# toverainc/willow-inference-server

Measured on NVIDIA H100. Metric: Whisper large-v2 realtime multiple (audio s / s), beam 5, 3.84 s utterance, higher is better.
Workload: dtype f16

## Files before the change

willow_inference_server_b200/csrc/decoder.cuh:

```cuda
#pragma once
#include "common.cuh"
#include "kernels.h"

namespace wisb {

constexpr int DEC_MAX_ROWS = 8;
constexpr int MAX_BEAM = 8;
constexpr int MAX_CAND = 2 * MAX_BEAM;
constexpr int TOPK_CHUNKS = 32;

struct DecState {
  int pos;
  int gen_step;
  int n_done;
  int all_done;
  int ticket;
};

enum GemvEpi : int {
  GV_STORE = 0,
  GV_RESID = 1,
  GV_GELU = 2,
  GV_QKV = 3,
};
// ... 114 lines not shown
  const float* next_g = nullptr;
};
struct MegaLayer {
  MegaGemv qkv, o, cq, co, fc1, fc2;
  const __half* ck = nullptr;
  const __half* cv = nullptr;
  __half* kcache = nullptr;
  __half* vcache = nullptr;
};
struct MegaArgs {
  const MegaLayer* layers = nullptr;
  int n_layers = 0;
  MegaGemv vocab;
  int with_logits = 0;
  int R = 0, d = 0, H = 0, n_utt = 0, beam = 0, t_max = 0;
  int pf_len = 0, pf_tok_stride = 0, pf_slot_stride = 0;
  const int* tokens = nullptr;
  const __half* tok_emb = nullptr;
  const float* pos_emb = nullptr;
  float* x = nullptr;
  float* q = nullptr;
  float* ctx = nullptr;
  __half* ctx16 = nullptr;
  __half* q16 = nullptr;
  __half* xn16 = nullptr;
  float* xstat = nullptr;
  const int* indir0 = nullptr;
  const int* indir1 = nullptr;
  const int* flip = nullptr;
  const DecState* st = nullptr;
  float* cross_part = nullptr;
  unsigned* cross_flags = nullptr;
  unsigned* flags = nullptr;
  unsigned* epoch_base = nullptr;
  int barrier_mode = 0;
  int tc = 0;
  int dbg = 0;
  int trace_cta = 0, trace_layer = 0, trace_cap = 0;
  unsigned long long* trace = nullptr;
};
size_t mega_flags_words();
int mega_k_chunks(int K);
void mega_chunk_major(const __half* src, __half* dst, int N, int K, cudaStream_t stream);
void mega_mma_image(const __half* src, __half* dst, int N, int K, int grid, cudaStream_t stream);
void mega_ln_fold(const __half* w, const float* g, const float* b, const float* bias, float* s2, float* biasf, int N, int K,
                  cudaStream_t stream);
void dec_pass_run(const MegaArgs& a, int num_sms, cudaStream_t stream);

void lang_probs_run(const float* logits, long long ldl, const int* lang_ids, int n_lang, int n_utt, int row_stride,
                    float* probs , cudaStream_t stream);

}
```

willow_inference_server_b200/csrc/decoder_mega.cu:

```cuda
#include <cooperative_groups.h>

#include "decoder.cuh"
#include "ptx.cuh"

namespace wisb {

namespace {

constexpr int MG_CONS_WARPS = 7;
constexpr int MG_CONS = MG_CONS_WARPS * 32;
constexpr int MG_THREADS = MG_CONS + 32;
constexpr int MG_KC_MAX = 1536;
constexpr int MG_STAGE_BYTES = 12 * MG_KC_MAX * 2;
constexpr int MG_NSTAGE = 2;
constexpr int MG_CA_KEYS_MAX = MG_STAGE_BYTES / 128;
constexpr int MG_SCRATCH = 29696;
constexpr int MG_SLOT_BYTES = MG_CONS_WARPS * 448 * 2;
constexpr int MG_LY_STRIDE = 704;
constexpr int MG_LY_BYTES = 2 * MG_LY_STRIDE;
constexpr int MG_RED_FLOATS = (2 * 2 + 1) * MG_CONS_WARPS * 32;
constexpr int MG_SMEM = MG_NSTAGE * MG_STAGE_BYTES + 1024 + MG_RED_FLOATS * 4 + 4224 + MG_SCRATCH + MG_SLOT_BYTES + MG_LY_BYTES;
static_assert(MG_SMEM <= 232448, "decoder pass: shared memory");
static_assert(sizeof(MegaLayer) % 16 == 0 && sizeof(MegaLayer) <= MG_LY_STRIDE, "layer descriptor is copied with 16-byte cp.async");
__host__ __device__ constexpr int mg_gp(int nr) { return 32 / nr < 6 ? 32 / nr : 6; }
// ... 831 lines not shown
  if (blockIdx.x == 0 && ctid == 0) {
    *A.epoch_base = epoch;
    A.epoch_base[8] = epoch * gridDim.x;
  }
}


constexpr int FUSED_B_OFF = 36864;
template <int NR>
struct MmaSmem {
  static constexpr int NS = NR <= 5 ? 4 : 3;
  static constexpr int B_BYTES = (5120 / 64) * NR * 128;
  static constexpr int B_MIN = FUSED_B_OFF + 20 * NR * 128;
  static constexpr int B_ALLOC = B_BYTES > B_MIN ? (B_BYTES > MG_SCRATCH ? B_BYTES : MG_SCRATCH) : (B_MIN > MG_SCRATCH ? B_MIN : MG_SCRATCH);
  static constexpr int OFF_B = NS * MG_STAGE_BYTES;
  static constexpr int OFF_PART = OFF_B + B_ALLOC;
  static constexpr int PART_BYTES = MG_CONS_WARPS * 8 * 68 * 4;
  static constexpr int OFF_BARS = OFF_PART + PART_BYTES;
  static constexpr int OFF_STAT = OFF_BARS + 256;
  static constexpr int OFF_SLOT = OFF_STAT + 4224;
  static constexpr int OFF_LY = OFF_SLOT + MG_SLOT_BYTES;
  static constexpr int OFF_GEOM = OFF_LY + MG_LY_BYTES;
  static constexpr int TOTAL = OFF_GEOM + 5 * 64;
  static constexpr int STAT_OFF = 24576;
  static_assert(TOTAL <= 232448, "warp-MMA decoder pass: shared memory");
  static_assert(20 * NR * 128 <= STAT_OFF && STAT_OFF + 160 * NR * 8 <= FUSED_B_OFF && FUSED_B_OFF + 20 * NR * 128 <= B_ALLOC,
                "statistics landing zone / fused-phase B operand");
};
constexpr int MM_GROUP_ROWS = 64;
constexpr int MM_PART_LD = 68;

struct MmaGeom {
  int lo, hi, rows_pad, n_full, tail;
  int units_full, kbu_full, units_tail, kbu_tail, pad[7];
};
static_assert(sizeof(MmaGeom) == 64, "geometry table stride");
__device__ __forceinline__ void mma_units(int rows, int kblocks, int& units, int& kbu) {
  const int max_kbu = MG_STAGE_BYTES / (rows * 128);
  units = (kblocks + max_kbu - 1) / max_kbu;
  kbu = (kblocks + units - 1) / units;
}
__device__ __forceinline__ MmaGeom mma_geom(int N, int K) {
  MmaGeom m;
  const int G = static_cast<int>(gridDim.x), b = static_cast<int>(blockIdx.x);
  const int base = N / G, rem = N - base * G;
  m.lo = b * base + min(b, rem);
  m.rows_pad = base + (b < rem ? 1 : 0);
  m.hi = m.lo + m.rows_pad;
  m.n_full = m.rows_pad / MM_GROUP_ROWS;
  m.tail = m.rows_pad - m.n_full * MM_GROUP_ROWS;
  m.units_full = m.kbu_full = m.units_tail = m.kbu_tail = 0;
  if (m.n_full > 0) mma_units(MM_GROUP_ROWS, K / 64, m.units_full, m.kbu_full);
  if (m.tail > 0) mma_units(m.tail, K / 64, m.units_tail, m.kbu_tail);
  return m;
}

template <int NS>
__device__ __forceinline__ void produce_gemv_mma(Ring& rg, const MegaGemv& g, const MmaGeom* s_geom, int dbg) {
  const MmaGeom mg = s_geom[g.shape];
  const int n_groups = mg.n_full + (mg.tail ? 1 : 0);
  const int kblocks = g.K / 64;
  const uint64_t pol = l2_policy_evict_first();
  for (int gi = 0; gi < n_groups; ++gi) {
    const bool full = gi < mg.n_full;
    const int rows = full ? MM_GROUP_ROWS : mg.tail;
    const int units = full ? mg.units_full : mg.units_tail, kbu = full ? mg.kbu_full : mg.kbu_tail;
    const __half* base = g.w + static_cast<long long>(mg.lo + gi * MM_GROUP_ROWS) * g.K;
    for (int u = 0; u < units; ++u) {
      const int kb0 = u * kbu, nkb = min(kbu, kblocks - kb0);
      const int st = rg.unit % NS;
      mbar_wait(rg.empty(st), ((rg.unit / NS) & 1u) ^ 1u);
      uint32_t bytes = static_cast<uint32_t>(nkb * rows * 128);
      if (dbg & 2) bytes = (bytes >> 2) & ~15u;
      mbar_arrive_expect_tx(rg.full(st), bytes);
      bulk_load_1d_hint(rg.data0 + st * MG_STAGE_BYTES, base + static_cast<long long>(kb0) * rows * 64, bytes, rg.full(st), pol);
      ++rg.unit;
    }
  }
}

// ... 29 lines not shown
#pragma unroll
    for (int ks = 0; ks < 4; ++ks) {
      uint32_t af[NMT][4], ag[NMT][4];
#pragma unroll
      for (int m = 0; m < NMT; ++m) {
        ldmatrix_x4(a_kb + sw[ks] + m * 2048, af[m]);
        ldmatrix_x4(a_kb + a_step + sw[ks] + m * 2048, ag[m]);
      }
#pragma unroll
      for (int m = 0; m < NMT; ++m) {
        mma_m16n8k16(acc[m], af[m], bf[2 * ks], bf[2 * ks + 1]);
        mma_m16n8k16(acc2[m], ag[m], bg[2 * ks], bg[2 * ks + 1]);
      }
    }
  }
  if (it < n_it) {
    const uint4 b01 = lds128(b_kb), b23 = lds128(b_kb + b_plane);
    const uint32_t bf[8] = {b01.x, b01.y, b01.z, b01.w, b23.x, b23.y, b23.z, b23.w};
#pragma unroll
    for (int ks = 0; ks < 4; ++ks) {
      uint32_t af[NMT][4];
#pragma unroll
      for (int m = 0; m < NMT; ++m) ldmatrix_x4(a_kb + sw[ks] + m * 2048, af[m]);
#pragma unroll
      for (int m = 0; m < NMT; ++m) mma_m16n8k16(acc[m], af[m], bf[2 * ks], bf[2 * ks + 1]);
    }
  }
#pragma unroll
  for (int m = 0; m < NMT; ++m)
#pragma unroll
    for (int i = 0; i < 4; ++i) acc[m][i] += acc2[m][i];
}

constexpr int SA_WARPS = 2;
__device__ __forceinline__ void consume_self_attn_mma(const MegaArgs& A, const MegaLayer& ly, int ctid, uint8_t* s_scr,
                                                   const unsigned short* s_slot_tab, int pos_dec, int flipv, int* s_tr) {
  const int lane = ctid & 31, warp = ctid >> 5;
  const int d = A.d, H = A.H, G = static_cast<int>(gridDim.x);
  const int n_tasks = A.R * H;
  const bool pf = A.pf_len > 0;
  trace_ev(A, ctid, s_tr, 20);
  if (warp >= SA_WARPS) return;
  const uint32_t sK = smem_u32(s_scr) + warp * 8192, sV = sK + 4096;
  const unsigned short* my_slots = s_slot_tab + warp * 448;
  const __half* kcache = ly.kcache;
  const __half* vcache = ly.vcache;
  const int gq = lane >> 2, tq = lane & 3;
  const int ld_key = lane >> 3, ld_c = lane & 7;
  const uint32_t lm_off = static_cast<uint32_t>(((lane & 7) + ((lane >> 3) & 1) * 8) * 128);
  const int lm_c = lane >> 4;
  for (int i = warp; i * G + static_cast<int>(blockIdx.x) < n_tasks; i += SA_WARPS) {
    const int task = i * G + static_cast<int>(blockIdx.x);
    const bool tab = i == warp;
    const int r = task / H, h = task - r * H;
    const int pos = pf ? r % A.pf_len : pos_dec;
    const int own = row_slot(A, r);
    const int* indir = (flipv ? A.indir1 : A.indir0) + static_cast<long long>(r) * A.t_max;
    uint32_t aq[4][2];
    {
      const __half* qr = A.q16 + (static_cast<long long>(h) * A.R + r) * HEAD_DIM + 2 * tq;
#pragma unroll
      for (int ks = 0; ks < 4; ++ks) {
        aq[ks][0] = gq == 0 ? __ldcg(reinterpret_cast<const unsigned*>(qr + 16 * ks)) : 0u;
        aq[ks][1] = gq == 0 ? __ldcg(reinterpret_cast<const unsigned*>(qr + 16 * ks + 8)) : 0u;
      }
    }
    float m_run = -INFINITY, l_run = 0.f;
    float o[8][4];
#pragma unroll
    for (int j = 0; j < 8; ++j)
#pragma unroll
      for (int q = 0; q < 4; ++q) o[j][q] = 0.f;
    for (int t0 = 0; t0 <= pos; t0 += 32) {
#pragma unroll
      for (int it = 0; it < 8; ++it) {
        const int key = it * 4 + ld_key;
        const int t = min(t0 + key, pos);
        int slot = own;
        if (!pf && t != pos) slot = tab ? static_cast<int>(my_slots[t]) : __ldcg(indir + t);
        const long long off = (static_cast<long long>(slot) * A.t_max + t) * d + h * HEAD_DIM + ld_c * 8;
        const uint32_t dst = key * 128 + ((ld_c ^ (key & 7)) << 4);
        cp_async16(sK + dst, kcache + off);
        cp_async16(sV + dst, vcache + off);
      }
      cp_async_wait_all();
      __syncwarp();
      trace_ev(A, ctid, s_tr, 21);
// ... 98 lines not shown
      if (rl.bytes2 != 0) bulk_load_1d(s_b_addr + stat_off, rl.src2, rl.bytes2, xbar);
    }
  }
  cons_sync();
  if (A.trace != nullptr && blockIdx.x == 0 && ctid == 0) A.trace[2 * (epoch - epoch0)] = globaltimer_ns();
}
__device__ __forceinline__ Reload gemv_reload(const MegaArgs& A, const MegaGemv& g, const MmaGeom* s_geom) {
  Reload rl;
  if (s_geom[g.shape].rows_pad != 0) {
    rl.src = g.x16;
    rl.bytes = static_cast<uint32_t>((g.K / 64) * A.R * 128);
    if (g.ln_s2 != nullptr) {
      rl.src2 = A.xstat;
      rl.bytes2 = static_cast<uint32_t>(gridDim.x * A.R * 8);
    }
  }
  return rl;
}


template <int NR>
__device__ __forceinline__ void consume_gemv_mma(Ring& rg, const MegaArgs& A, const MegaGemv& g_mem, const MegaLayer* ly, int ctid,
                                             uint8_t* s_b, float* s_lnstat, float* s_mpart, float* s_xown, int* s_tr,
                                             const MmaGeom* s_geom, uint32_t xbar, unsigned& x_count) {
  using SM = MmaSmem<NR>;
  constexpr int NS = SM::NS;
  const MegaGemv g = g_mem;
  const MmaGeom mg = s_geom[g.shape];
  if (mg.rows_pad == 0) return;
  const int lane = ctid & 31, warp = ctid >> 5;
  const int R = A.R;
  const int kblocks = g.K / 64;
  const bool ln = g.ln_s2 != nullptr;
  const int G = static_cast<int>(gridDim.x);
  trace_ev(A, ctid, s_tr, 1);
  constexpr int NSLOT = (NR * MM_GROUP_ROWS + MG_CONS - 1) / MG_CONS;
  const int n_groups = mg.n_full + (mg.tail ? 1 : 0);
  const int first_rows = mg.n_full > 0 ? MM_GROUP_ROWS : mg.tail;
  const int wsh = (n_groups == 1 && first_rows <= 16) ? 4 : 6;
  float e_bias[NSLOT], e_s2[NSLOT], e_gain[NSLOT];
  auto prefetch_epi = [&](int gi, int rows) {
#pragma unroll
    for (int j = 0; j < NSLOT; ++j) {
      const int idx = ctid + j * MG_CONS;
      const int m = idx & ((1 << wsh) - 1), n = mg.lo + gi * MM_GROUP_ROWS + m;
      const bool ok = (idx >> wsh) < R && m < rows && n < mg.hi;
      e_bias[j] = (ok && g.bias != nullptr) ? __ldg(g.bias + n) : 0.f;
      e_s2[j] = (ok && ln) ? __ldg(g.ln_s2 + n) : 0.f;
      e_gain[j] = (ok && g.next_g != nullptr) ? __ldg(g.next_g + n) : 0.f;
    }
  };
  prefetch_epi(0, first_rows);
  const int gq = lane >> 2, tq = lane & 3;
  const int brow = gq < R ? gq : R - 1;
  const uint32_t b_lane = smem_u32(s_b) + (brow * 4 + tq) * 16, b_plane = static_cast<uint32_t>(R * 64);
  const int a_row = (lane & 7) + ((lane >> 3) & 1) * 8;
  uint32_t sw[4];
#pragma unroll
  for (int ks = 0; ks < 4; ++ks) sw[ks] = ((2 * ks + (lane >> 4)) ^ (a_row & 7)) << 4;
  const uint32_t a_lane = rg.data0 + a_row * 128;
  unsigned unit = rg.unit;
  unsigned st = unit % NS, par = (unit / NS) & 1u;
  mbar_wait(xbar, x_count & 1u);
  ++x_count;
  trace_ev(A, ctid, s_tr, 2);
  for (int gi = 0; gi < n_groups; ++gi) {
    const bool full = gi < mg.n_full;
    const int rows = full ? MM_GROUP_ROWS : mg.tail;
    const int n_mt = (rows + 15) >> 4;
    const int units = full ? mg.units_full : mg.units_tail, kbu = full ? mg.kbu_full : mg.kbu_tail;
    if (gi > 0) prefetch_epi(gi, rows);
    float acc[4][4];
#pragma unroll
    for (int m = 0; m < 4; ++m)
#pragma unroll
      for (int i = 0; i < 4; ++i) acc[m][i] = 0.f;
    int kb_next = warp;
    for (int u = 0, kb0 = 0; u < units; ++u, kb0 += kbu) {
      const int nkb = min(kbu, kblocks - kb0);
      mbar_wait(rg.full(st), par);
      if (u == 0 && gi == 0) trace_ev(A, ctid, s_tr, 3);
// ... 45 lines not shown
    for (int j = 0; j < NSLOT; ++j) {
      const int idx = ctid + j * MG_CONS;
      const int r = idx >> wsh, m = idx & ((1 << wsh) - 1);
      const int n = mg.lo + gi * MM_GROUP_ROWS + m;
      const bool valid = r < R && m < rows && n < mg.hi;
      float v = 0.f;
      if (valid) {
#pragma unroll
        for (int w = 0; w < MG_CONS_WARPS; ++w) v += s_mpart[(w * 8 + r) * MM_PART_LD + m];
        if (ln) {
          const float mean = s_lnstat[2 * r] / g.K;
          const float rstd = rsqrtf(fmaxf(s_lnstat[2 * r + 1] / g.K - mean * mean, 0.f) + 1e-5f);
          v = rstd * (v - mean * e_s2[j]);
        }
        v += e_bias[j];
      }
      if (g.epi == GV_RESID) {
        float nv = 0.f;
        if (valid) {
          nv = s_xown[r * 16 + (n - mg.lo)] + v;
          s_xown[r * 16 + (n - mg.lo)] = nv;
        }
        if (j == 0 || (idx >> 5) * 32 < R * 16) publish_resid(A, r, n, valid, nv, e_gain[j], lane);
      } else if (valid) {
        switch (g.epi) {
          case GV_STORE:
            if (g.out16 != nullptr) g.out16[(static_cast<long long>(n >> 6) * R + r) * HEAD_DIM + (n & 63)] = __float2half_rn(v * 0.125f);
            else g.out[static_cast<long long>(r) * g.ldo + n] = v;
            break;
          case GV_GELU:
            g.out16[act16_off(R, r, n)] = __float2half_rn(gelu_erf(v));
            break;
          case GV_QKV: {
            const int d = A.d;
            if (n < d) {
              A.q16[(static_cast<long long>(n >> 6) * R + r) * HEAD_DIM + (n & 63)] = __float2half_rn(v * 0.125f);
            } else {
              const int pos = row_pos(A, r);
              __half* cache = (n < 2 * d) ? ly->kcache : ly->vcache;
              const int e = (n < 2 * d) ? n - d : n - 2 * d;
              cache[(static_cast<long long>(row_slot(A, r)) * A.t_max + pos) * d + e] = __float2half_rn(v);
            }
            break;
          }
          default:
            break;
        }
      }
    }
    if (gi + 1 < n_groups) cons_sync();
  }
  trace_ev(A, ctid, s_tr, 6);
  rg.unit = unit;
}

template <int NS>
__device__ __forceinline__ void produce_cross_fused(Ring& rg, const MegaArgs& A, const MegaLayer& ly, const MmaGeom* s_geom) {
  const CrossGeom cg = cross_geom(A.n_utt, A.H);
  const uint64_t pol = l2_policy_evict_first();
  const int kblocks = A.d / 64, units = s_geom[4].units_full, kbu = s_geom[4].kbu_full;
  for (int task = blockIdx.x; task < cg.n_tasks; task += gridDim.x) {
    const int split = task % cg.S, uh = task / cg.S;
    const int h = uh % A.H;
    const __half* wq = ly.cq.w + static_cast<long long>(h) * 64 * A.d;
    for (int u = 0; u < units; ++u) {
      const int kb0 = u * kbu, nkb = min(kbu, kblocks - kb0);
      const int st = rg.unit % NS;
      mbar_wait(rg.empty(st), ((rg.unit / NS) & 1u) ^ 1u);
      mbar_arrive_expect_tx(rg.full(st), static_cast<uint32_t>(nkb * 64 * 128));
      bulk_load_1d_hint(rg.data0 + st * MG_STAGE_BYTES, wq + static_cast<long long>(kb0) * 64 * 64, static_cast<uint32_t>(nkb * 64 * 128),
                        rg.full(st), pol);
      ++rg.unit;
    }
// ... 217 lines not shown
  extern __shared__ __align__(1024) uint8_t mg_smem[];
  uint8_t* s_b = mg_smem + SM::OFF_B;
  float* s_part = reinterpret_cast<float*>(s_b);
  float* s_mpart = reinterpret_cast<float*>(mg_smem + SM::OFF_PART);
  uint64_t* bars = reinterpret_cast<uint64_t*>(mg_smem + SM::OFF_BARS);
  float* s_stat = reinterpret_cast<float*>(mg_smem + SM::OFF_STAT);
  float* s_lnstat = s_stat;
  unsigned short* s_slot_tab = reinterpret_cast<unsigned short*>(mg_smem + SM::OFF_SLOT);
  MegaLayer* s_ly = reinterpret_cast<MegaLayer*>(mg_smem + SM::OFF_LY);
  MmaGeom* s_geom = reinterpret_cast<MmaGeom*>(mg_smem + SM::OFF_GEOM);
  float* s_xown = s_stat + 784;
  int* s_tr = reinterpret_cast<int*>(s_stat + 16);
  Ring rg;
  rg.data = mg_smem;
  rg.data0 = smem_u32(mg_smem);
  rg.full0 = smem_u32(bars);
  rg.empty0 = rg.full0 + 8 * NS;
  rg.unit = 0;
  const uint32_t xbar = rg.full0 + 8 * (2 * NS);
  unsigned x_count = 0;
  const int tid = threadIdx.x;
  if ((smem_u32(mg_smem) & 1023u) != 0) __trap();
  if (tid == 0) {
    for (int s = 0; s < NS; ++s) {
      mbar_init(rg.full(s), 1);
      mbar_init(rg.empty(s), MG_CONS_WARPS);
    }
    mbar_init(xbar, 1);
    fence_mbar_init();
  }
  if (tid < 5) {
    const int d = A.d;
    const int Ns[5] = {3 * d, d, 4 * d, d, A.vocab.N}, Ks[5] = {d, d, d, 4 * d, d};
    s_geom[tid] = mma_geom(Ns[tid], Ks[tid]);
  }
  __syncthreads();
  const int L = A.n_layers;

  if (tid >= MG_CONS) {
    if (tid == MG_CONS) {
      for (int l = 0; l <= L; ++l) {
        if (l == L) {
          if (A.with_logits) produce_gemv_mma<NS>(rg, A.vocab, s_geom, A.dbg);
          break;
        }
        const MegaLayer& ly = A.layers[l];
        for (int j = 0; j < 6; ++j) {
          if (j == 2) produce_cross_fused<NS>(rg, A, ly, s_geom);
          else produce_gemv_mma<NS>(rg, (&ly.qkv)[j], s_geom, A.dbg);
        }
      }
    }
    return;
  }
  const int ctid = tid;
  unsigned epoch = *A.epoch_base;
  const unsigned epoch0 = epoch;
  if (ctid == 0) s_tr[0] = -1;
  if (A.trace != nullptr && blockIdx.x == 0 && ctid == 0) A.trace[0] = globaltimer_ns();
  auto prefetch_layer = [&](int l) {
    if (ctid < static_cast<int>(sizeof(MegaLayer) / 16))
      cp_async16(smem_u32(reinterpret_cast<uint8_t*>(s_ly) + (l & 1) * MG_LY_STRIDE) + ctid * 16,
                 reinterpret_cast<const uint8_t*>(A.layers + l) + ctid * 16);
  };
  if (L > 0) prefetch_layer(0);
  const int pos_dec = A.pf_len > 0 ? 0 : A.st->pos;
  const int flipv = *A.flip;
  if (A.pf_len == 0 && (ctid >> 5) < SA_WARPS) {
    const int task = (ctid >> 5) * static_cast<int>(gridDim.x) + static_cast<int>(blockIdx.x);
    if (task < A.R * A.H) {
      const int* indir = (flipv ? A.indir1 : A.indir0) + static_cast<long long>(task / A.H) * A.t_max;
      for (int t = ctid & 31; t < pos_dec; t += 32) s_slot_tab[(ctid >> 5) * 448 + t] = static_cast<unsigned short>(indir[t]);
    }
  }
  cp_async_wait_all();
  {
    const MmaGeom mg = s_geom[1];
    const float* gain0 = L > 0 ? A.layers[0].qkv.ln_g : A.vocab.ln_g;
    for (int base = 0; base < A.R * 16; base += MG_CONS) {
      const int idx = base + ctid;
      const int r = idx >> 4, c = idx & 15, n = mg.lo + c;
      const bool valid = r < A.R && n < mg.hi;
      float v = 0.f, gain = 0.f;
      if (valid) {
        v = __half2float(A.tok_emb[static_cast<long long>(row_token(A, r)) * A.d + n]) + A.pos_emb[static_cast<long long>(row_pos(A, r)) * A.d + n];
        gain = __ldg(gain0 + n);
        s_xown[r * 16 + c] = v;
      }
      if ((idx >> 5) * 32 < A.R * 16) publish_resid(A, r, n, valid, v, gain, ctid & 31);
    }
  }
  const uint32_t sba = smem_u32(s_b);
  Reload rl_next = L > 0 ? gemv_reload(A, A.layers[0].qkv, s_geom) : (A.with_logits ? gemv_reload(A, A.vocab, s_geom) : Reload());
  for (int l = -1; l <= L; ++l) {
    const bool vocab_layer = l == L;
    if (vocab_layer && !A.with_logits) break;
    const MegaLayer& ly = *reinterpret_cast<const MegaLayer*>(reinterpret_cast<const uint8_t*>(s_ly) + ((l < 0 ? 0 : l) & 1) * MG_LY_STRIDE);
    if (l >= 0 && l + 1 < L) prefetch_layer(l + 1);
    if (l >= 0) trace_open(A, ctid, s_tr, l);
    const int n_ph = (l < 0 || vocab_layer) ? 1 : 7;
    for (int ph = 0; ph < n_ph; ++ph) {
      if (l < 0) {
      } else if (!vocab_layer && ph == 1) {
        consume_self_attn_mma(A, ly, ctid, reinterpret_cast<uint8_t*>(s_part), s_slot_tab, pos_dec, flipv, s_tr);
      } else if (!vocab_layer && ph == 3) {
        consume_cross_fused<NR, NS>(rg, A, ly, ctid, s_b, s_mpart, s_lnstat, s_tr, s_geom, xbar, x_count, epoch + 1, SM::STAT_OFF);
      } else {
        const MegaGemv& g = vocab_layer ? A.vocab : (&ly.qkv)[ph == 0 ? 0 : (ph == 2 ? 1 : ph - 1)];
        consume_gemv_mma<NR>(rg, A, g, &ly, ctid, s_b, s_lnstat, s_mpart, s_xown, s_tr, s_geom, xbar, x_count);
      }
      Reload rl = rl_next;
      if (l >= 0) {
        rl = Reload();
        if (!vocab_layer) {
          if (ph == 6) {
            cp_async_wait_all();
            rl = l + 1 < L ? gemv_reload(A, ly.qkv, s_geom) : (A.with_logits ? gemv_reload(A, A.vocab, s_geom) : Reload());
          } else if (ph == 2) {
            rl.src = ly.cq.x16;
            rl.bytes = static_cast<uint32_t>((A.d / 64) * A.R * 128);
            rl.src2 = A.xstat;
            rl.bytes2 = static_cast<uint32_t>(gridDim.x * A.R * 8);
            rl.dst_off = FUSED_B_OFF;
          } else if (ph != 0) {
            rl = gemv_reload(A, (&ly.qkv)[ph == 1 ? 1 : ph], s_geom);
          }
        }
      }
      grid_barrier_mma(A, epoch, ctid, epoch0, rl, sba, SM::STAT_OFF, xbar, s_tr);
    }
  }
  trace_dump(A, ctid, s_tr);
  if (blockIdx.x == 0 && ctid == 0) {
    *A.epoch_base = epoch;
    A.epoch_base[8] = epoch * gridDim.x;
  }
}

__global__ void chunk_major_kernel(const __half* __restrict__ src, __half* __restrict__ dst, int N, int K, int n_chunks) {
  const int kc = K / n_chunks;
  const long long total = static_cast<long long>(N) * K / 8;
  for (long long i = blockIdx.x * static_cast<long long>(blockDim.x) + threadIdx.x; i < total; i += static_cast<long long>(gridDim.x) * blockDim.x) {
    const long long e = i * 8;
    const int n = static_cast<int>(e / K), k = static_cast<int>(e - static_cast<long long>(n) * K);
    const int c = k / kc, kk = k - c * kc;
    *reinterpret_cast<uint4*>(dst + (static_cast<long long>(c) * N + n) * kc + kk) = *reinterpret_cast<const uint4*>(src + e);
  }
}

__global__ void mma_image_kernel(const __half* __restrict__ src, __half* __restrict__ dst, int N, int K, int G) {
  const int base = N / G, rem = N - base * G;
  const int big = rem * (base + 1);
  const int kc = K >> 3;
  const long long total = static_cast<long long>(N) * kc;
  for (long long i = blockIdx.x * static_cast<long long>(blockDim.x) + threadIdx.x; i < total; i += static_cast<long long>(gridDim.x) * blockDim.x) {
    const int n = static_cast<int>(i / kc), c16 = static_cast<int>(i - static_cast<long long>(n) * kc);
    int lo, rows;
    if (n < big) {
      rows = base + 1;
      lo = (n / rows) * rows;
    } else {
      rows = base;
      lo = big + ((n - big) / rows) * rows;
    }
    const int rl = n - lo, gi = rl >> 6, row = rl & 63;
    const int rows_g = min(64, rows - gi * 64);
    const int kb = c16 >> 3, c = c16 & 7;
    const uint4 v = *reinterpret_cast<const uint4*>(src + static_cast<long long>(n) * K + c16 * 8);
    *reinterpret_cast<uint4*>(dst + static_cast<long long>(lo + gi * 64) * K + static_cast<long long>(kb) * rows_g * 64 + row * 64 + ((c ^ (row & 7)) << 3)) = v;
  }
}

}

void mega_mma_image(const __half* src, __half* dst, int N, int K, int grid, cudaStream_t stream) {
  mma_image_kernel<<<1024, 256, 0, stream>>>(src, dst, N, K, grid);
  WISB_CUDA(cudaGetLastError());
}

__global__ void ln_fold_kernel(const __half* __restrict__ w, const float* __restrict__ g, const float* __restrict__ b,
                               const float* __restrict__ bias, float* __restrict__ s2, float* __restrict__ biasf, int N, int K) {
  const int n = blockIdx.x * (blockDim.x >> 5) + (threadIdx.x >> 5);
  const int lane = threadIdx.x & 31;
  if (n >= N) return;
  float a = 0.f, c = 0.f;
  for (int k = lane; k < K; k += 32) {
    const float wv = __half2float(w[static_cast<long long>(n) * K + k]);
    a = fmaf(g[k], wv, a);
    c = fmaf(b[k], wv, c);
  }
  a = warp_sum(a);
  c = warp_sum(c);
  if (lane == 0) {
    s2[n] = a;
    biasf[n] = c + (bias != nullptr ? bias[n] : 0.f);
  }
}

void mega_ln_fold(const __half* w, const float* g, const float* b, const float* bias, float* s2, float* biasf, int N, int K,
                  cudaStream_t stream) {
  ln_fold_kernel<<<cdiv(N, 8), 256, 0, stream>>>(w, g, b, bias, s2, biasf, N, K);
  WISB_CUDA(cudaGetLastError());
}

int mega_k_chunks(int K) {
  int n = (K + MG_KC_MAX - 1) / MG_KC_MAX;
  while (K % (8 * n) != 0) ++n;
  return n;
}
// ... 46 lines not shown
```

willow_inference_server_b200/csrc/engine.cu:

```cuda
#include <stdio.h>
#include <string.h>

#include <algorithm>
#include <functional>
#include <map>
#include <memory>
#include <mutex>
#include <string>
#include <vector>

#include "../../include/wisb200.h"
#include "decoder.cuh"
#include "kernels.h"

namespace wisb {

namespace {

thread_local std::string g_last_error;

struct TensorRef {
  const uint8_t* ptr = nullptr;
  int dtype = 0, ndim = 0;
  long long shape[4] = {1, 1, 1, 1};
// ... 85 lines not shown
  int mel_B = 0;
  int enc_cap = 0;
  DevBuf<__half> h1, xn, qkv, vt, ctx, hbuf, enc_out, ckv;
  DevBuf<float> x;
  GemmPlan plan_conv2, plan_ckv;
  CUtensorMap ckv_map;
  std::vector<EncLayerPlans> enc_plans;
  AttnPlan attn_plan;
  int plans_B = 0, plans_vmn = -1, plans_pdl = -1;
  DevBuf<float> dx, dq, dctx, dh, logits;
  DevBuf<__half> dctx16, dh16, dxn16, dq16;
  DevBuf<float> dxstat;
  DevBuf<__half> kcache, vcache;
  DevBuf<uint8_t> mask_base, mask_cur;
  std::vector<int> mask_extra;
  DevBuf<float> row_lse, cum, cand_score, best_score, lang_probs, part_max, part_sum;
  DevBuf<unsigned long long> part;
  DevBuf<int> cand_idx, tokens, seq0, seq1, ind0, ind1, flip, done, n_hyp, best_len, best_tokens, prompt_dev, lang_ids;
  DevBuf<DecState> st;
  DevBuf<int> row_pos, row_slot, max_new_u;
  int search_rows = 0;
  int search_gen = 0, bd_search_gen = -1;
  int batch_rows = 320, batch_pdl = 1, decoder_batch = 1, mega_barrier = 1, cross_tc = 1, debug_chunk = 1;
  int bd_rows = 0, bd_tcap = 0, bd_launches_step = 0;
  DevBuf<float> bx, bq, bpart, blogits;
  DevBuf<__half> bxn, bctx, bh, bkc, bvc;
  std::vector<BatchLayer> bd_layers;
  GemmPlan bd_vocab;
  DevBuf<MegaLayer> mega_layers;
  DevBuf<__half> mega_img;
  int enc_pdl = 1;
  int mega_tc = 1, mega_dbg = 0;
  DevBuf<unsigned> mega_flags;
  int encoder_cache = 0;
  std::vector<float> mel_cache;
  int mel_cache_B = 0;
  bool enc_valid = false;
  int ckv_is_sw = 0;
  DevBuf<float> cross_part;
  DevBuf<unsigned> cross_flags;
  DevBuf<float> ln_fold;
  DevBuf<__half> fc2_chunked;
  std::vector<int> al_layer_off;
  int al_A = 0;
  DevBuf<int> al_items, al_head, al_ntext, al_nframes, al_text, al_path, al_len;
  DevBuf<float> al_cap, al_mat, al_probs;
  DevBuf<unsigned long long> mega_trace;
  int mega_trace_on = 0, mega_trace_cta = 0, mega_trace_layer = 0;
  cudaEvent_t ev_flag[2] = {nullptr, nullptr};
  PinBuf<MegaLayer> mega_layers_host;
  PinBuf<int> pin_i;
  PinBuf<float> pin_f;
  PinBuf<uint8_t> pin_b;
  std::map<GraphKey, cudaGraphExec_t> graphs;
  cudaEvent_t ev[8] = {};
  float timing[16] = {};
  int launches = 0;
  int profile = 0;
  std::vector<cudaEvent_t> prof_ev;
  std::vector<int> prof_cat;
  size_t prof_used = 0;
  void prof_begin(int cat) {
    if (!profile) return;
    if (prof_used + 2 > prof_ev.size()) {
      cudaEvent_t a, b;
      WISB_CUDA(cudaEventCreate(&a));
// ... 220 lines not shown
    }
    h->al_layer_off[d.n_dec_layers] = A;
    for (int a = 0; a < A; ++a) heads[a] = lh[2 * a + 1];
    h->al_A = A;
    h->al_items.ensure(A);
    h->al_head.ensure(A);
    WISB_CUDA(cudaMemcpy(h->al_items.p, items.data(), A * 4, cudaMemcpyHostToDevice));
    WISB_CUDA(cudaMemcpy(h->al_head.p, heads.data(), A * 4, cudaMemcpyHostToDevice));
  }
  h->mask_base.ensure(d.n_vocab);
  h->mask_cur.ensure(d.n_vocab);
  WISB_CUDA(cudaMemcpy(h->mask_base.p, mask.data(), mask.size(), cudaMemcpyHostToDevice));
  WISB_CUDA(cudaMemcpy(h->mask_cur.p, mask.data(), mask.size(), cudaMemcpyHostToDevice));
  const size_t R = DEC_MAX_ROWS;
  h->dx.ensure(R * d.d_model, true);
  h->dq.ensure(R * d.d_model, true);
  h->dctx.ensure(R * d.d_model, true);
  h->dh.ensure(R * 4 * d.d_model, true);
  h->dctx16.ensure(R * d.d_model, true);
  h->dh16.ensure(R * 4 * d.d_model, true);
  h->dxn16.ensure(R * d.d_model, true);
  h->dq16.ensure(R * d.d_model, true);
  h->dxstat.ensure(static_cast<size_t>(h->num_sms) * R * 2, true);
  h->logits.ensure(R * d.n_vocab_pad, true);
  const size_t cache = static_cast<size_t>(d.n_dec_layers) * R * T_MAX * d.d_model;
  h->kcache.ensure(cache, true);
  h->vcache.ensure(cache, true);
  h->flip.ensure(1, true);
  h->st.ensure(1, true);
  ensure_search(h, DEC_MAX_ROWS);
  h->mega_layers.ensure(d.n_dec_layers);
  h->mega_layers_host.ensure(d.n_dec_layers);
  h->mega_flags.ensure(mega_flags_words(), true);
  h->cross_flags.ensure(static_cast<size_t>(DEC_MAX_ROWS) * d.n_heads * 16 * 32, true);
  {
    const size_t per_layer = 2ull * (3 * d.d_model + d.d_model + 4 * d.d_model);
    h->ln_fold.ensure(per_layer * d.n_dec_layers + 2ull * d.n_vocab_pad);
    for (int i = 0; i < d.n_dec_layers; ++i) {
      const DecLayerW& w = h->dec_w[i];
      float* base = h->ln_fold.p + per_layer * i;
      mega_ln_fold(w.qkvw, w.ln1g, w.ln1b, w.qkvb, base, base + 3 * d.d_model, 3 * d.d_model, d.d_model, h->stream);
      base += 6 * d.d_model;
      mega_ln_fold(w.cqw, w.ln2g, w.ln2b, w.cqb, base, base + d.d_model, d.d_model, d.d_model, h->stream);
      base += 2 * d.d_model;
      mega_ln_fold(w.fc1w, w.ln3g, w.ln3b, w.fc1b, base, base + 4 * d.d_model, 4 * d.d_model, d.d_model, h->stream);
    }
    float* vb = h->ln_fold.p + per_layer * d.n_dec_layers;
    mega_ln_fold(h->H("dec.tok_emb"), h->F("dec.ln.g"), h->F("dec.ln.b"), nullptr, vb, vb + d.n_vocab_pad, d.n_vocab, d.d_model, h->stream);
  }
  if (mega_k_chunks(4 * d.d_model) > 1) {
    const size_t per = static_cast<size_t>(4) * d.d_model * d.d_model;
    h->fc2_chunked.ensure(per * d.n_dec_layers);
    for (int i = 0; i < d.n_dec_layers; ++i)
      mega_chunk_major(h->dec_w[i].fc2w, h->fc2_chunked.p + per * i, d.d_model, 4 * d.d_model, h->stream);
  }
  h->cross_part.ensure(static_cast<size_t>(DEC_MAX_ROWS) * d.n_heads * 16 * MAX_BEAM * 68, true);
  if (4 * d.d_model <= 5120 && d.d_model % 64 == 0) {
    const size_t dd = d.d_model;
    const size_t per_layer = 14 * dd * dd;
    const size_t vocab_rows = static_cast<size_t>(d.n_vocab);
    h->mega_img.ensure(per_layer * d.n_dec_layers + vocab_rows * dd);
    for (int i = 0; i < d.n_dec_layers; ++i) {
      const DecLayerW& w = h->dec_w[i];
      __half* p = h->mega_img.p + per_layer * i;
      mega_mma_image(w.qkvw, p, 3 * d.d_model, d.d_model, h->num_sms, h->stream);
      mega_mma_image(w.ow, p + 3 * dd * dd, d.d_model, d.d_model, h->num_sms, h->stream);
      mega_mma_image(w.cqw, p + 4 * dd * dd, d.d_model, d.d_model, d.n_heads, h->stream);
      mega_mma_image(w.cow, p + 5 * dd * dd, d.d_model, d.d_model, h->num_sms, h->stream);
      mega_mma_image(w.fc1w, p + 6 * dd * dd, 4 * d.d_model, d.d_model, h->num_sms, h->stream);
      mega_mma_image(w.fc2w, p + 10 * dd * dd, d.d_model, 4 * d.d_model, h->num_sms, h->stream);
    }
    mega_mma_image(h->H("dec.tok_emb"), h->mega_img.p + per_layer * d.n_dec_layers, d.n_vocab, d.d_model, h->num_sms, h->stream);
  } else {
    h->mega_tc = 0;
  }
  WISB_CUDA(cudaStreamSynchronize(h->stream));
}

size_t mel_floats(const wisb_handle* h, int B) { return static_cast<size_t>(B) * h->dims.n_mels * N_FRAMES; }

void ensure_mel(wisb_handle* h, int B) {
  h->lm_max.ensure(B);
  const size_t n = mel_floats(h, B);
  if (n <= h->mel.n) return;
  h->mel.ensure(n);
  h->mel_B = 0;
}

void ensure_encoder(wisb_handle* h, int B) {
  if (h->blob == nullptr) return;
  const Dims& dm = h->dims;
  const int d = dm.d_model, H = dm.n_heads;
  const long long M = static_cast<long long>(B) * T_ENC_PAD;
  if (B > h->enc_cap) {
    h->plans_B = 0;
    drop_graphs(h);
    h->h1.release();
    h->h1.ensure((static_cast<size_t>(B) * H1_ROWS + 8) * d, true);
    h->x.ensure(M * d, true);
    h->xn.ensure(M * d, true);
    h->qkv.ensure(M * 3 * d, true);
    h->vt.ensure(M * d, true);
    h->ctx.ensure(M * d, true);
    h->hbuf.ensure(M * 4 * d, true);
    h->enc_out.ensure(M * d, true);
// ... 343 lines not shown
    a.q16 = h->dq16.p;
    a.xstat = h->dxstat.p;
    a.vocab.x16 = h->dxn16.p;
    a.vocab.shape = 4;
  }
  a.with_logits = with_logits ? 1 : 0;
  a.R = c.n_utt * c.beam;
  a.d = dm.d_model;
  a.H = dm.n_heads;
  a.n_utt = c.n_utt;
  a.beam = c.beam;
  a.t_max = T_MAX;
  a.tokens = h->tokens.p;
  if (prefill_pass) {
    a.pf_len = c.prompt_len - 1;
    a.pf_tok_stride = c.prompt_len;
    a.pf_slot_stride = c.beam;
    a.R = c.n_utt * a.pf_len;
    a.beam = a.pf_len;
    a.tokens = h->prompt_dev.p;
  }
  a.tok_emb = h->H("dec.tok_emb");
  a.pos_emb = h->F("dec.pos");
  a.x = h->dx.p;
  a.q = h->dq.p;
  a.ctx = h->dctx.p;
  a.indir0 = h->ind0.p;
  a.indir1 = h->ind1.p;
  a.flip = h->flip.p;
  a.st = h->st.p;
  a.cross_part = h->cross_part.p;
  a.cross_flags = h->cross_flags.p;
  a.flags = h->mega_flags.p;
  a.epoch_base = h->mega_flags.p + 160 * 32;
  a.barrier_mode = h->mega_barrier;
  if (h->mega_trace_on) {
    h->mega_trace.ensure(2048 + 160 * 264, true);
    a.trace = h->mega_trace.p;
    a.trace_cta = h->mega_trace_cta;
    a.trace_layer = h->mega_trace_layer;
    a.trace_cap = h->mega_tc ? 380 : 70;
  }
  dec_pass_run(a, h->num_sms, h->stream);
}

void enqueue_prefill(wisb_handle* h, const DecodeCfg& c) {
  enqueue_decoder_forward(h, c, false);
  prefill_advance_run(h->tokens.p, h->prompt_dev.p, c.prompt_len, c.n_utt * c.beam, c.beam, h->st.p, h->stream);
}
void enqueue_step(wisb_handle* h, const DecodeCfg& c) {
  enqueue_decoder_forward(h, c, true);
  search_step_run(make_search_args(h, c), h->stream);
}

void set_extra_suppress(wisb_handle* h, const int32_t* extra, int n_extra) {
  std::vector<int> want(extra ? extra : nullptr, extra ? extra + n_extra : nullptr);
  if (want == h->mask_extra) return;
  const Dims& dm = h->dims;
  for (int id : want) WISB_REQUIRE(id >= 0 && id < dm.n_vocab, "suppress token id outside the vocabulary");
  h->mask_extra.assign(1, -1);
  WISB_CUDA(cudaMemcpyAsync(h->mask_cur.p, h->mask_base.p, dm.n_vocab, cudaMemcpyDeviceToDevice, h->stream));
  if (!want.empty()) {
    std::vector<uint8_t> m(dm.n_vocab);
    WISB_CUDA(cudaMemcpyAsync(m.data(), h->mask_base.p, dm.n_vocab, cudaMemcpyDeviceToHost, h->stream));
    WISB_CUDA(cudaStreamSynchronize(h->stream));
    for (int id : want) m[id] |= 1;
// ... 1565 lines not shown
```

Baseline: 129.2.

## Group QKV rows per head so self-attention runs after local head handoff

Reorders the QKV weight image so each group of CTAs owns the q, k and v rows of a single attention head. Self-attention for that head can then start once only its group has finished, signalled through per-CTA head flags, rather than after a grid-wide phase barrier. This removes one global barrier per decoder layer, cutting the phase count from seven to six. In exchange it adds spin-waits on the new flags, remaps QKV rows for bias, LN-fold and epilogue lookups, and requires at least as many SMs as heads.

```diff
diff --git a/willow_inference_server_b200/csrc/decoder.cuh b/willow_inference_server_b200/csrc/decoder.cuh
--- a/willow_inference_server_b200/csrc/decoder.cuh
+++ b/willow_inference_server_b200/csrc/decoder.cuh
@@ -170,6 +170,7 @@
   float* cross_part = nullptr;
   unsigned* cross_flags = nullptr;
   unsigned* flags = nullptr;
+  unsigned* head_flags = nullptr;
   unsigned* epoch_base = nullptr;
   int barrier_mode = 0;
   int tc = 0;
@@ -180,7 +181,7 @@
 size_t mega_flags_words();
 int mega_k_chunks(int K);
 void mega_chunk_major(const __half* src, __half* dst, int N, int K, cudaStream_t stream);
-void mega_mma_image(const __half* src, __half* dst, int N, int K, int grid, cudaStream_t stream);
+void mega_mma_image(const __half* src, __half* dst, int N, int K, int grid, int qkv_heads, cudaStream_t stream);
 void mega_ln_fold(const __half* w, const float* g, const float* b, const float* bias, float* s2, float* biasf, int N, int K,
                   cudaStream_t stream);
 void dec_pass_run(const MegaArgs& a, int num_sms, cudaStream_t stream);
diff --git a/willow_inference_server_b200/csrc/decoder_mega.cu b/willow_inference_server_b200/csrc/decoder_mega.cu
--- a/willow_inference_server_b200/csrc/decoder_mega.cu
+++ b/willow_inference_server_b200/csrc/decoder_mega.cu
@@ -887,20 +887,44 @@
 
 struct MmaGeom {
   int lo, hi, rows_pad, n_full, tail;
-  int units_full, kbu_full, units_tail, kbu_tail, pad[7];
+  int units_full, kbu_full, units_tail, kbu_tail;
+  int head, grp_lo, grp_n;
+  int pad[4];
 };
 static_assert(sizeof(MmaGeom) == 64, "geometry table stride");
+__device__ __forceinline__ void deal(int n, int parts, int i, int& lo, int& cnt) {
+  const int base = n / parts, rem = n - base * parts;
+  lo = i * base + min(i, rem);
+  cnt = base + (i < rem ? 1 : 0);
+}
+__device__ __forceinline__ int deal_part(int n, int parts, int k) {
+  const int base = n / parts, rem = n - base * parts, big = rem * (base + 1);
+  return k < big ? k / (base + 1) : rem + (k - big) / base;
+}
+__device__ __forceinline__ void mma_own(int N, int G, int heads, int b, int& lo, int& cnt, int& head, int& grp_lo, int& grp_n) {
+  head = grp_lo = grp_n = 0;
+  if (heads == 0) {
+    deal(N, G, b, lo, cnt);
+    return;
+  }
+  const int P = N / heads;
+  head = deal_part(G, heads, b);
+  deal(G, heads, head, grp_lo, grp_n);
+  deal(P, grp_n, b - grp_lo, lo, cnt);
+  lo += head * P;
+}
+__device__ __forceinline__ int qkv_src_row(int n, int d) {
+  const int h = n / (3 * HEAD_DIM), j = n - h * 3 * HEAD_DIM;
+  return (j >> 6) * d + h * HEAD_DIM + (j & 63);
+}
 __device__ __forceinline__ void mma_units(int rows, int kblocks, int& units, int& kbu) {
   const int max_kbu = MG_STAGE_BYTES / (rows * 128);
   units = (kblocks + max_kbu - 1) / max_kbu;
   kbu = (kblocks + units - 1) / units;
 }
-__device__ __forceinline__ MmaGeom mma_geom(int N, int K) {
+__device__ __forceinline__ MmaGeom mma_geom(int N, int K, int heads) {
   MmaGeom m;
-  const int G = static_cast<int>(gridDim.x), b = static_cast<int>(blockIdx.x);
-  const int base = N / G, rem = N - base * G;
-  m.lo = b * base + min(b, rem);
-  m.rows_pad = base + (b < rem ? 1 : 0);
+  mma_own(N, static_cast<int>(gridDim.x), heads, static_cast<int>(blockIdx.x), m.lo, m.rows_pad, m.head, m.grp_lo, m.grp_n);
   m.hi = m.lo + m.rows_pad;
   m.n_full = m.rows_pad / MM_GROUP_ROWS;
   m.tail = m.rows_pad - m.n_full * MM_GROUP_ROWS;
@@ -996,12 +1020,24 @@
     for (int i = 0; i < 4; ++i) acc[m][i] += acc2[m][i];
 }
 
+__device__ __forceinline__ void head_handoff(const MegaArgs& A, const MmaGeom& mg, int ctid, unsigned tag, int* s_tr) {
+  cons_sync();
+  if (ctid == 0) st_release_gpu(A.head_flags + blockIdx.x * 32, tag);
+  if (static_cast<int>(blockIdx.x) - mg.grp_lo >= A.R) return;
+  if (ctid < mg.grp_n) {
+    const unsigned* f = A.head_flags + (mg.grp_lo + ctid) * 32;
+    while (ld_acquire_gpu(f) != tag) {
+    }
+  }
+  cons_sync();
+  trace_ev(A, ctid, s_tr, 25);
+}
+
 constexpr int SA_WARPS = 2;
-__device__ __forceinline__ void consume_self_attn_mma(const MegaArgs& A, const MegaLayer& ly, int ctid, uint8_t* s_scr,
+__device__ __forceinline__ void consume_self_attn_mma(const MegaArgs& A, const MegaLayer& ly, const MmaGeom& mg, int ctid, uint8_t* s_scr,
                                                    const unsigned short* s_slot_tab, int pos_dec, int flipv, int* s_tr) {
   const int lane = ctid & 31, warp = ctid >> 5;
-  const int d = A.d, H = A.H, G = static_cast<int>(gridDim.x);
-  const int n_tasks = A.R * H;
+  const int d = A.d, h = mg.head, lb = static_cast<int>(blockIdx.x) - mg.grp_lo;
   const bool pf = A.pf_len > 0;
   trace_ev(A, ctid, s_tr, 20);
   if (warp >= SA_WARPS) return;
@@ -1013,10 +1049,9 @@
   const int ld_key = lane >> 3, ld_c = lane & 7;
   const uint32_t lm_off = static_cast<uint32_t>(((lane & 7) + ((lane >> 3) & 1) * 8) * 128);
   const int lm_c = lane >> 4;
-  for (int i = warp; i * G + static_cast<int>(blockIdx.x) < n_tasks; i += SA_WARPS) {
-    const int task = i * G + static_cast<int>(blockIdx.x);
+  for (int i = warp; lb + i * mg.grp_n < A.R; i += SA_WARPS) {
+    const int r = lb + i * mg.grp_n;
     const bool tab = i == warp;
-    const int r = task / H, h = task - r * H;
     const int pos = pf ? r % A.pf_len : pos_dec;
     const int own = row_slot(A, r);
     const int* indir = (flipv ? A.indir1 : A.indir0) + static_cast<long long>(r) * A.t_max;
@@ -1181,6 +1216,7 @@
   const int R = A.R;
   const int kblocks = g.K / 64;
   const bool ln = g.ln_s2 != nullptr;
+  const bool qkv = g.epi == GV_QKV;
   const int G = static_cast<int>(gridDim.x);
   trace_ev(A, ctid, s_tr, 1);
   constexpr int NSLOT = (NR * MM_GROUP_ROWS + MG_CONS - 1) / MG_CONS;
@@ -1194,8 +1230,9 @@
       const int idx = ctid + j * MG_CONS;
       const int m = idx & ((1 << wsh) - 1), n = mg.lo + gi * MM_GROUP_ROWS + m;
       const bool ok = (idx >> wsh) < R && m < rows && n < mg.hi;
-      e_bias[j] = (ok && g.bias != nullptr) ? __ldg(g.bias + n) : 0.f;
-      e_s2[j] = (ok && ln) ? __ldg(g.ln_s2 + n) : 0.f;
+      const int ns = qkv ? qkv_src_row(n, A.d) : n;
+      e_bias[j] = (ok && g.bias != nullptr) ? __ldg(g.bias + ns) : 0.f;
+      e_s2[j] = (ok && ln) ? __ldg(g.ln_s2 + ns) : 0.f;
       e_gain[j] = (ok && g.next_g != nullptr) ? __ldg(g.next_g + n) : 0.f;
     }
   };
@@ -1307,13 +1344,13 @@
             g.out16[act16_off(R, r, n)] = __float2half_rn(gelu_erf(v));
             break;
           case GV_QKV: {
-            const int d = A.d;
-            if (n < d) {
-              A.q16[(static_cast<long long>(n >> 6) * R + r) * HEAD_DIM + (n & 63)] = __float2half_rn(v * 0.125f);
+            const int d = A.d, ns = qkv_src_row(n, d);
+            if (ns < d) {
+              A.q16[(static_cast<long long>(ns >> 6) * R + r) * HEAD_DIM + (ns & 63)] = __float2half_rn(v * 0.125f);
             } else {
               const int pos = row_pos(A, r);
-              __half* cache = (n < 2 * d) ? ly->kcache : ly->vcache;
-              const int e = (n < 2 * d) ? n - d : n - 2 * d;
+              __half* cache = (ns < 2 * d) ? ly->kcache : ly->vcache;
+              const int e = (ns < 2 * d) ? ns - d : ns - 2 * d;
               cache[(static_cast<long long>(row_slot(A, r)) * A.t_max + pos) * d + e] = __float2half_rn(v);
             }
             break;
@@ -1597,7 +1634,7 @@
   if (tid < 5) {
     const int d = A.d;
     const int Ns[5] = {3 * d, d, 4 * d, d, A.vocab.N}, Ks[5] = {d, d, d, 4 * d, d};
-    s_geom[tid] = mma_geom(Ns[tid], Ks[tid]);
+    s_geom[tid] = mma_geom(Ns[tid], Ks[tid], tid == 0 ? A.H : 0);
   }
   __syncthreads();
   const int L = A.n_layers;
@@ -1632,9 +1669,9 @@
   const int pos_dec = A.pf_len > 0 ? 0 : A.st->pos;
   const int flipv = *A.flip;
   if (A.pf_len == 0 && (ctid >> 5) < SA_WARPS) {
-    const int task = (ctid >> 5) * static_cast<int>(gridDim.x) + static_cast<int>(blockIdx.x);
-    if (task < A.R * A.H) {
-      const int* indir = (flipv ? A.indir1 : A.indir0) + static_cast<long long>(task / A.H) * A.t_max;
+    const int r = static_cast<int>(blockIdx.x) - s_geom[0].grp_lo + (ctid >> 5) * s_geom[0].grp_n;
+    if (r < A.R) {
+      const int* indir = (flipv ? A.indir1 : A.indir0) + static_cast<long long>(r) * A.t_max;
       for (int t = ctid & 31; t < pos_dec; t += 32) s_slot_tab[(ctid >> 5) * 448 + t] = static_cast<unsigned short>(indir[t]);
     }
   }
@@ -1663,32 +1700,35 @@
     const MegaLayer& ly = *reinterpret_cast<const MegaLayer*>(reinterpret_cast<const uint8_t*>(s_ly) + ((l < 0 ? 0 : l) & 1) * MG_LY_STRIDE);
     if (l >= 0 && l + 1 < L) prefetch_layer(l + 1);
     if (l >= 0) trace_open(A, ctid, s_tr, l);
-    const int n_ph = (l < 0 || vocab_layer) ? 1 : 7;
+    const int n_ph = (l < 0 || vocab_layer) ? 1 : 6;
     for (int ph = 0; ph < n_ph; ++ph) {
       if (l < 0) {
-      } else if (!vocab_layer && ph == 1) {
-        consume_self_attn_mma(A, ly, ctid, reinterpret_cast<uint8_t*>(s_part), s_slot_tab, pos_dec, flipv, s_tr);
-      } else if (!vocab_layer && ph == 3) {
+      } else if (!vocab_layer && ph == 2) {
         consume_cross_fused<NR, NS>(rg, A, ly, ctid, s_b, s_mpart, s_lnstat, s_tr, s_geom, xbar, x_count, epoch + 1, SM::STAT_OFF);
       } else {
-        const MegaGemv& g = vocab_layer ? A.vocab : (&ly.qkv)[ph == 0 ? 0 : (ph == 2 ? 1 : ph - 1)];
+        const MegaGemv& g = vocab_layer ? A.vocab : (&ly.qkv)[ph];
         consume_gemv_mma<NR>(rg, A, g, &ly, ctid, s_b, s_lnstat, s_mpart, s_xown, s_tr, s_geom, xbar, x_count);
+        if (!vocab_layer && ph == 0) {
+          const MmaGeom mg = s_geom[0];
+          head_handoff(A, mg, ctid, epoch + 1, s_tr);
+          consume_self_attn_mma(A, ly, mg, ctid, reinterpret_cast<uint8_t*>(s_part), s_slot_tab, pos_dec, flipv, s_tr);
+        }
       }
       Reload rl = rl_next;
       if (l >= 0) {
         rl = Reload();
         if (!vocab_layer) {
-          if (ph == 6) {
+          if (ph == 5) {
             cp_async_wait_all();
             rl = l + 1 < L ? gemv_reload(A, ly.qkv, s_geom) : (A.with_logits ? gemv_reload(A, A.vocab, s_geom) : Reload());
-          } else if (ph == 2) {
+          } else if (ph == 1) {
             rl.src = ly.cq.x16;
             rl.bytes = static_cast<uint32_t>((A.d / 64) * A.R * 128);
             rl.src2 = A.xstat;
             rl.bytes2 = static_cast<uint32_t>(gridDim.x * A.R * 8);
             rl.dst_off = FUSED_B_OFF;
-          } else if (ph != 0) {
-            rl = gemv_reload(A, (&ly.qkv)[ph == 1 ? 1 : ph], s_geom);
+          } else {
+            rl = gemv_reload(A, (&ly.qkv)[ph + 1], s_geom);
           }
         }
       }
@@ -1713,33 +1753,34 @@
   }
 }
 
-__global__ void mma_image_kernel(const __half* __restrict__ src, __half* __restrict__ dst, int N, int K, int G) {
-  const int base = N / G, rem = N - base * G;
-  const int big = rem * (base + 1);
+__global__ void mma_image_kernel(const __half* __restrict__ src, __half* __restrict__ dst, int N, int K, int G, int qkv_heads) {
   const int kc = K >> 3;
   const long long total = static_cast<long long>(N) * kc;
   for (long long i = blockIdx.x * static_cast<long long>(blockDim.x) + threadIdx.x; i < total; i += static_cast<long long>(gridDim.x) * blockDim.x) {
     const int n = static_cast<int>(i / kc), c16 = static_cast<int>(i - static_cast<long long>(n) * kc);
-    int lo, rows;
-    if (n < big) {
-      rows = base + 1;
-      lo = (n / rows) * rows;
+    int lo, rows, head, grp_lo, grp_n, b;
+    if (qkv_heads > 0) {
+      const int P = N / qkv_heads, h = n / P;
+      deal(G, qkv_heads, h, grp_lo, grp_n);
+      b = grp_lo + deal_part(P, grp_n, n - h * P);
     } else {
-      rows = base;
-      lo = big + ((n - big) / rows) * rows;
-    }
+      b = deal_part(N, G, n);
+    }
+    mma_own(N, G, qkv_heads, b, lo, rows, head, grp_lo, grp_n);
     const int rl = n - lo, gi = rl >> 6, row = rl & 63;
     const int rows_g = min(64, rows - gi * 64);
     const int kb = c16 >> 3, c = c16 & 7;
-    const uint4 v = *reinterpret_cast<const uint4*>(src + static_cast<long long>(n) * K + c16 * 8);
+    const int n_src = qkv_heads > 0 ? qkv_src_row(n, N / 3) : n;
+    const uint4 v = *reinterpret_cast<const uint4*>(src + static_cast<long long>(n_src) * K + c16 * 8);
     *reinterpret_cast<uint4*>(dst + static_cast<long long>(lo + gi * 64) * K + static_cast<long long>(kb) * rows_g * 64 + row * 64 + ((c ^ (row & 7)) << 3)) = v;
   }
 }
 
 }
 
-void mega_mma_image(const __half* src, __half* dst, int N, int K, int grid, cudaStream_t stream) {
-  mma_image_kernel<<<1024, 256, 0, stream>>>(src, dst, N, K, grid);
+void mega_mma_image(const __half* src, __half* dst, int N, int K, int grid, int qkv_heads, cudaStream_t stream) {
+  WISB_REQUIRE(qkv_heads == 0 || (N == 3 * qkv_heads * HEAD_DIM && grid >= qkv_heads), "QKV image: one CTA group per head");
+  mma_image_kernel<<<1024, 256, 0, stream>>>(src, dst, N, K, grid, qkv_heads);
   WISB_CUDA(cudaGetLastError());
 }
 
diff --git a/willow_inference_server_b200/csrc/engine.cu b/willow_inference_server_b200/csrc/engine.cu
--- a/willow_inference_server_b200/csrc/engine.cu
+++ b/willow_inference_server_b200/csrc/engine.cu
@@ -141,6 +141,7 @@
   int enc_pdl = 1;
   int mega_tc = 1, mega_dbg = 0;
   DevBuf<unsigned> mega_flags;
+  DevBuf<unsigned> head_flags;
   int encoder_cache = 0;
   std::vector<float> mel_cache;
   int mel_cache_B = 0;
@@ -427,6 +428,7 @@
   h->mega_layers.ensure(d.n_dec_layers);
   h->mega_layers_host.ensure(d.n_dec_layers);
   h->mega_flags.ensure(mega_flags_words(), true);
+  h->head_flags.ensure(mega_flags_words(), true);
   h->cross_flags.ensure(static_cast<size_t>(DEC_MAX_ROWS) * d.n_heads * 16 * 32, true);
   {
     const size_t per_layer = 2ull * (3 * d.d_model + d.d_model + 4 * d.d_model);
@@ -450,7 +452,7 @@
       mega_chunk_major(h->dec_w[i].fc2w, h->fc2_chunked.p + per * i, d.d_model, 4 * d.d_model, h->stream);
   }
   h->cross_part.ensure(static_cast<size_t>(DEC_MAX_ROWS) * d.n_heads * 16 * MAX_BEAM * 68, true);
-  if (4 * d.d_model <= 5120 && d.d_model % 64 == 0) {
+  if (4 * d.d_model <= 5120 && d.d_model % 64 == 0 && h->num_sms >= d.n_heads) {
     const size_t dd = d.d_model;
     const size_t per_layer = 14 * dd * dd;
     const size_t vocab_rows = static_cast<size_t>(d.n_vocab);
@@ -458,14 +460,14 @@
     for (int i = 0; i < d.n_dec_layers; ++i) {
       const DecLayerW& w = h->dec_w[i];
       __half* p = h->mega_img.p + per_layer * i;
-      mega_mma_image(w.qkvw, p, 3 * d.d_model, d.d_model, h->num_sms, h->stream);
-      mega_mma_image(w.ow, p + 3 * dd * dd, d.d_model, d.d_model, h->num_sms, h->stream);
-      mega_mma_image(w.cqw, p + 4 * dd * dd, d.d_model, d.d_model, d.n_heads, h->stream);
-      mega_mma_image(w.cow, p + 5 * dd * dd, d.d_model, d.d_model, h->num_sms, h->stream);
-      mega_mma_image(w.fc1w, p + 6 * dd * dd, 4 * d.d_model, d.d_model, h->num_sms, h->stream);
-      mega_mma_image(w.fc2w, p + 10 * dd * dd, d.d_model, 4 * d.d_model, h->num_sms, h->stream);
-    }
-    mega_mma_image(h->H("dec.tok_emb"), h->mega_img.p + per_layer * d.n_dec_layers, d.n_vocab, d.d_model, h->num_sms, h->stream);
+      mega_mma_image(w.qkvw, p, 3 * d.d_model, d.d_model, h->num_sms, d.n_heads, h->stream);
+      mega_mma_image(w.ow, p + 3 * dd * dd, d.d_model, d.d_model, h->num_sms, 0, h->stream);
+      mega_mma_image(w.cqw, p + 4 * dd * dd, d.d_model, d.d_model, d.n_heads, 0, h->stream);
+      mega_mma_image(w.cow, p + 5 * dd * dd, d.d_model, d.d_model, h->num_sms, 0, h->stream);
+      mega_mma_image(w.fc1w, p + 6 * dd * dd, 4 * d.d_model, d.d_model, h->num_sms, 0, h->stream);
+      mega_mma_image(w.fc2w, p + 10 * dd * dd, d.d_model, 4 * d.d_model, h->num_sms, 0, h->stream);
+    }
+    mega_mma_image(h->H("dec.tok_emb"), h->mega_img.p + per_layer * d.n_dec_layers, d.n_vocab, d.d_model, h->num_sms, 0, h->stream);
   } else {
     h->mega_tc = 0;
   }
@@ -875,6 +877,7 @@
   a.cross_part = h->cross_part.p;
   a.cross_flags = h->cross_flags.p;
   a.flags = h->mega_flags.p;
+  a.head_flags = h->head_flags.p;
   a.epoch_base = h->mega_flags.p + 160 * 32;
   a.barrier_mode = h->mega_barrier;
   if (h->mega_trace_on) {
```

New measurement: 129.8, median of 6. Within noise of the previous version (+0.5%).
